# seceq/zkir

Hardware: AMD Instinct MI355X
Metric: trace rows/sec (2^20-cycle fib: execution-trace fill + BabyBear NTT/LDE + Poseidon2 Merkle commitment) (higher is better)
Workload: dtype u32 (Baby Bear, 31-bit modular) / u64 trace words

## Files before the change

### zkir_amd/csrc/babybear.h

```cpp
#pragma once
#include <cstdint>

#if defined(__HIPCC__)
#define BB_HD __host__ __device__ __forceinline__
#else
#define BB_HD inline
#endif

namespace bb {

constexpr uint32_t P = 0x78000001u;
constexpr uint32_t NEG_PINV = 0x77FFFFFFu;
constexpr uint32_t R1 = 0x0FFFFFFEu;
constexpr uint32_t R2 = 0x45DDDDE3u;
constexpr uint32_t GEN = 31u;
constexpr uint32_t ROOT27 = 0x1A427A41u;
constexpr uint32_t W_EXT = 11u;

BB_HD uint32_t add(uint32_t a, uint32_t b) { const uint32_t s = a + b, d = s - P; return d < s ? d : s; }
BB_HD uint32_t sub(uint32_t a, uint32_t b) { const uint32_t d = a - b, e = d + P; return e < d ? e : d; }
BB_HD uint32_t neg(uint32_t a) { return a ? P - a : 0u; }
BB_HD uint32_t dbl(uint32_t a) { return add(a, a); }
BB_HD uint32_t mont_mul(uint32_t a, uint32_t b) {
  const uint64_t t = (uint64_t)a * b;
// ... 179 lines not shown
      "v_mad_i64_i32 %2, vcc, %11, %16, %3\n\tv_mad_i64_i32 %6, vcc, %15, %16, %7\n\t"
      "v_mad_i64_i32 %1, vcc, %9, %17, %1\n\tv_mad_i64_i32 %5, vcc, %13, %17, %5\n\t"
      "v_mad_i64_i32 %3, vcc, %11, %17, %3\n\tv_mad_i64_i32 %7, vcc, %15, %17, %7"
      : "=&v"(ay0), "=&v"(ay1), "=&v"(at2), "=&v"(at3), "=&v"(by0), "=&v"(by1), "=&v"(bt2), "=&v"(bt3)
      : "v"(a[0]), "v"(a[1]), "v"(a[2]), "v"(a[3]), "v"(b[0]), "v"(b[1]), "v"(b[2]), "v"(b[3]), "v"(w1), "v"(n1), "s"(W_ONE) : "vcc");
  {
    const int32_t m0 = (int32_t)((uint32_t)at2 * NEG_PINV), m1 = (int32_t)((uint32_t)bt2 * NEG_PINV), m2 = (int32_t)((uint32_t)at3 * NEG_PINV), m3 = (int32_t)((uint32_t)bt3 * NEG_PINV);
    asm("v_mad_i64_i32 %0, vcc, %4, %8, %0\n\tv_mad_i64_i32 %1, vcc, %5, %8, %1\n\tv_mad_i64_i32 %2, vcc, %6, %8, %2\n\tv_mad_i64_i32 %3, vcc, %7, %8, %3"
        : "+v"(at2), "+v"(bt2), "+v"(at3), "+v"(bt3) : "v"(m0), "v"(m1), "v"(m2), "v"(m3), "s"((int32_t)P) : "vcc");
  }
  const int32_t ay2 = (int32_t)((uint64_t)at2 >> 32), ay3 = (int32_t)((uint64_t)at3 >> 32), by2 = (int32_t)((uint64_t)bt2 >> 32), by3 = (int32_t)((uint64_t)bt3 >> 32);
  int64_t au0, au1, bu0, bu1;
  asm("v_mad_i64_i32 %0, vcc, %8, %12, %4\n\tv_mad_i64_i32 %2, vcc, %10, %12, %6\n\t"
      "v_mad_i64_i32 %1, vcc, %9, %14, %5\n\tv_mad_i64_i32 %3, vcc, %11, %14, %7\n\t"
      "v_mad_i64_i32 %4, vcc, %8, %13, %4\n\tv_mad_i64_i32 %6, vcc, %10, %13, %6\n\t"
      "v_mad_i64_i32 %5, vcc, %9, %15, %5\n\tv_mad_i64_i32 %7, vcc, %11, %15, %7"
      : "=&v"(au0), "=&v"(au1), "=&v"(bu0), "=&v"(bu1), "+v"(ay0), "+v"(ay1), "+v"(by0), "+v"(by1)
      : "v"(ay2), "v"(ay3), "v"(by2), "v"(by3), "v"(w2), "v"(n2), "v"(w2i), "v"(n2i) : "vcc");
  {
    const int32_t m0 = (int32_t)((uint32_t)au0 * NEG_PINV), m1 = (int32_t)((uint32_t)bu0 * NEG_PINV), m2 = (int32_t)((uint32_t)au1 * NEG_PINV), m3 = (int32_t)((uint32_t)bu1 * NEG_PINV);
    const int32_t m4 = (int32_t)((uint32_t)ay0 * NEG_PINV), m5 = (int32_t)((uint32_t)by0 * NEG_PINV), m6 = (int32_t)((uint32_t)ay1 * NEG_PINV), m7 = (int32_t)((uint32_t)by1 * NEG_PINV);
    asm("v_mad_i64_i32 %0, vcc, %8, %16, %0\n\tv_mad_i64_i32 %1, vcc, %9, %16, %1\n\tv_mad_i64_i32 %2, vcc, %10, %16, %2\n\tv_mad_i64_i32 %3, vcc, %11, %16, %3\n\t"
        "v_mad_i64_i32 %4, vcc, %12, %16, %4\n\tv_mad_i64_i32 %5, vcc, %13, %16, %5\n\tv_mad_i64_i32 %6, vcc, %14, %16, %6\n\tv_mad_i64_i32 %7, vcc, %15, %16, %7"
        : "+v"(au0), "+v"(bu0), "+v"(au1), "+v"(bu1), "+v"(ay0), "+v"(by0), "+v"(ay1), "+v"(by1)
        : "v"(m0), "v"(m1), "v"(m2), "v"(m3), "v"(m4), "v"(m5), "v"(m6), "v"(m7), "s"((int32_t)P) : "vcc");
  }
  a[0] = (int32_t)((uint64_t)au0 >> 32); a[1] = (int32_t)((uint64_t)au1 >> 32); a[2] = (int32_t)((uint64_t)ay0 >> 32); a[3] = (int32_t)((uint64_t)ay1 >> 32);
  b[0] = (int32_t)((uint64_t)bu0 >> 32); b[1] = (int32_t)((uint64_t)bu1 >> 32); b[2] = (int32_t)((uint64_t)by0 >> 32); b[3] = (int32_t)((uint64_t)by1 >> 32);
#else
  dit4w(a[0], a[1], a[2], a[3], w1, n1, w2, n2, w2i, n2i);
  dit4w(b[0], b[1], b[2], b[3], w1, n1, w2, n2, w2i, n2i);
#endif
}
constexpr uint64_t WREDC_IN_MAX = (1ull << 63) - ((uint64_t)P << 31);
constexpr uint64_t wredc_out_bound(uint64_t acc) { return (acc >> 32) + 1 + P / 2 + 1; }
struct WBound { uint64_t acc, out; };
constexpr WBound dit2w_bound(uint64_t x) { const uint64_t a = x * (uint64_t)W_ONE + x * (uint64_t)W_HALF; return WBound{a, wredc_out_bound(a)}; }
constexpr WBound dit4w_bound(uint64_t x) {
  const uint64_t s1 = x * (uint64_t)W_ONE + x * (uint64_t)W_HALF;
  const uint64_t s2 = s1 + wredc_out_bound(s1) * (uint64_t)W_HALF;
  return WBound{s2, wredc_out_bound(s2)};
}
static_assert(dit4w_bound(1ull << 31).acc < WREDC_IN_MAX && dit2w_bound(1ull << 31).acc < WREDC_IN_MAX, "every sum of a quad on int32 words is a legal reduction input");
static_assert(dit4w_bound(1ull << 31).out < (1ull << 31) && dit2w_bound(1ull << 31).out < (1ull << 31), "any quad output (and any canonical word) is a legal quad input");
static_assert(dit4w_bound(P).out < P && dit2w_bound(P).out < P, "closure: words in (-p, p) -- canonical ones included -- stay in (-p, p), which is what wcanon() takes");

BB_HD uint32_t to_mont(uint32_t a) { return mont_mul(a, R2); }
BB_HD uint32_t from_mont(uint32_t a) { return mont_mul(a, 1u); }
BB_HD uint32_t mul(uint32_t a, uint32_t b) { return mont_mul(mont_mul(a, b), R2); }
BB_HD uint32_t pow(uint32_t a, uint64_t e) {
  uint32_t r = R1, b = to_mont(a);
  while (e) { if (e & 1) r = mont_mul(r, b); b = mont_mul(b, b); e >>= 1; }
  return from_mont(r);
}
BB_HD uint32_t inv(uint32_t a) { return pow(a, P - 2); }
BB_HD uint32_t root_of_unity(int log_n) { uint32_t w = ROOT27; for (int i = log_n; i < 27; i++) w = mul(w, w); return w; }

struct E4 { uint32_t c[4]; };
BB_HD E4 e_add(const E4& a, const E4& b) { return E4{{add(a.c[0], b.c[0]), add(a.c[1], b.c[1]), add(a.c[2], b.c[2]), add(a.c[3], b.c[3])}}; }
BB_HD E4 e_sub(const E4& a, const E4& b) { return E4{{sub(a.c[0], b.c[0]), sub(a.c[1], b.c[1]), sub(a.c[2], b.c[2]), sub(a.c[3], b.c[3])}}; }
BB_HD E4 e_mul_m(const E4& a, const E4& b) {
  constexpr uint32_t W11M = (uint32_t)((11ull * R1) % P);
  const uint32_t a0 = a.c[0], a1 = a.c[1], a2 = a.c[2], a3 = a.c[3], b0 = b.c[0], b1 = b.c[1], b2 = b.c[2], b3 = b.c[3];
  const uint32_t t4 = add(add(mont_mul(a1, b3), mont_mul(a2, b2)), mont_mul(a3, b1));
  const uint32_t t5 = add(mont_mul(a2, b3), mont_mul(a3, b2));
  const uint32_t t6 = mont_mul(a3, b3);
  E4 r;
  r.c[0] = add(mont_mul(a0, b0), mont_mul(W11M, t4));
  r.c[1] = add(add(mont_mul(a0, b1), mont_mul(a1, b0)), mont_mul(W11M, t5));
  r.c[2] = add(add(add(mont_mul(a0, b2), mont_mul(a1, b1)), mont_mul(a2, b0)), mont_mul(W11M, t6));
  r.c[3] = add(add(mont_mul(a0, b3), mont_mul(a1, b2)), add(mont_mul(a2, b1), mont_mul(a3, b0)));
  return r;
}
BB_HD E4 e_mul_fm(const E4& a, uint32_t bm) { return E4{{mont_mul(a.c[0], bm), mont_mul(a.c[1], bm), mont_mul(a.c[2], bm), mont_mul(a.c[3], bm)}}; }
BB_HD E4 e_to_mont(const E4& a) { return E4{{to_mont(a.c[0]), to_mont(a.c[1]), to_mont(a.c[2]), to_mont(a.c[3])}}; }
BB_HD E4 e_from_mont(const E4& a) { return E4{{from_mont(a.c[0]), from_mont(a.c[1]), from_mont(a.c[2]), from_mont(a.c[3])}}; }
BB_HD E4 e_one_m() { return E4{{R1, 0, 0, 0}}; }
BB_HD E4 e_zero() { return E4{{0, 0, 0, 0}}; }
// ... 17 lines not shown
```

### zkir_amd/csrc/ntt.hip

```cpp
#include <hip/hip_runtime.h>

#include <atomic>
#include <cstdlib>
#include <mutex>
#include <type_traits>

#include "../../include/zkir_amd.h"
#include "../../include/zkir_amd_experimental.h"
#include "babybear.h"
#include "host.h"

namespace {

constexpr int NT = 256;
__device__ __forceinline__ uint32_t bitrev(uint32_t x, int bits) { return bits == 0 ? 0u : __brev(x) >> (32 - bits); }

template <int K, int N, class F>
__device__ __forceinline__ void static_for(F&& f) {
  if constexpr (K < N) { f(std::integral_constant<int, K>{}); static_for<K + 1, N>(f); }
}

using u32x4 = uint32_t __attribute__((ext_vector_type(4)));
__device__ __forceinline__ u32x4 ld4(const uint4* p) { return *reinterpret_cast<const u32x4*>(p); }
__device__ __forceinline__ void st4(uint4* p, u32x4 v) { *reinterpret_cast<u32x4*>(p) = v; }

__device__ __forceinline__ void wave_sync_lds() { asm volatile("s_waitcnt lgkmcnt(0)" ::: "memory"); }

__device__ __forceinline__ uint4 add4(uint4 a, uint4 b) { return make_uint4(bb::add(a.x, b.x), bb::add(a.y, b.y), bb::add(a.z, b.z), bb::add(a.w, b.w)); }
__device__ __forceinline__ uint4 subl4(uint4 a, uint4 b) { return make_uint4(a.x - b.x + bb::P, a.y - b.y + bb::P, a.z - b.z + bb::P, a.w - b.w + bb::P); }
__device__ __forceinline__ uint4 mul4(uint4 a, uint32_t w) { return make_uint4(bb::mont_mul(a.x, w), bb::mont_mul(a.y, w), bb::mont_mul(a.z, w), bb::mont_mul(a.w, w)); }

__device__ __forceinline__ void dif4(uint4& x0, uint4& x1, uint4& x2, uint4& x3, uint32_t wA, uint32_t wB, uint32_t w2) {
  const uint4 y0 = add4(x0, x2), y2 = mul4(subl4(x0, x2), wA);
  const uint4 y1 = add4(x1, x3), y3 = mul4(subl4(x1, x3), wB);
  x0 = add4(y0, y1); x1 = mul4(subl4(y0, y1), w2);
  x2 = add4(y2, y3); x3 = mul4(subl4(y2, y3), w2);
}

struct WTw { int32_t w, n; };
__device__ __forceinline__ WTw wtw(int32_t w) { return WTw{w, -w}; }
__device__ __forceinline__ void dit4w4(uint4& x0, uint4& x1, uint4& x2, uint4& x3, WTw w1, WTw w2, WTw w2i) {
#define ZKIR_Q(c, e) { int32_t a[4] = {(int32_t)x0.c, (int32_t)x1.c, (int32_t)x2.c, (int32_t)x3.c}, b[4] = {(int32_t)x0.e, (int32_t)x1.e, (int32_t)x2.e, (int32_t)x3.e}; \
                       bb::dit4w2(a, b, w1.w, w1.n, w2.w, w2.n, w2i.w, w2i.n); \
                       x0.c = (uint32_t)a[0]; x1.c = (uint32_t)a[1]; x2.c = (uint32_t)a[2]; x3.c = (uint32_t)a[3]; x0.e = (uint32_t)b[0]; x1.e = (uint32_t)b[1]; x2.e = (uint32_t)b[2]; x3.e = (uint32_t)b[3]; }
  ZKIR_Q(x, y) __builtin_amdgcn_sched_barrier(0); ZKIR_Q(z, w)
#undef ZKIR_Q
}
__device__ __forceinline__ void dit2w4(uint4& a, uint4& b, WTw w) {
#define ZKIR_Q(c) { int32_t p = (int32_t)a.c, q = (int32_t)b.c; bb::dit2w(p, q, w.w, w.n); a.c = (uint32_t)p; b.c = (uint32_t)q; }
  ZKIR_Q(x) ZKIR_Q(y) ZKIR_Q(z) ZKIR_Q(w)
#undef ZKIR_Q
}
__device__ __forceinline__ uint4 canon4(uint4 v) { return make_uint4(bb::wcanon((int32_t)v.x), bb::wcanon((int32_t)v.y), bb::wcanon((int32_t)v.z), bb::wcanon((int32_t)v.w)); }

template <bool DIT>
__global__ __launch_bounds__(NT) void ntt_stage_kernel(uint4* __restrict__ data, uint64_t blk_u4, int L, int s0, const uint32_t* __restrict__ tw, int canon) {
  uint4* x = data + (uint64_t)blockIdx.y * blk_u4;
  const uint64_t item = (uint64_t)blockIdx.x * NT + threadIdx.x;
  const uint32_t n = 1u << L;
  if (item >= (uint64_t)n) return;
  const uint32_t t = (uint32_t)(item >> 1), h = (uint32_t)(item & 1);
  uint32_t p, stride, w;
  if (DIT) { stride = 1u << s0; const uint32_t hi = t >> s0, lo = t & (stride - 1); p = (hi << (s0 + 1)) + lo; w = tw[lo << (L - s0 - 1)]; }
  else { stride = n >> (s0 + 1); const uint32_t hi = t / stride, lo = t % stride; p = hi * (n >> s0) + lo; w = tw[lo << s0]; }
  const uint4 a = x[(uint64_t)p * 2 + h], b = x[(uint64_t)(p + stride) * 2 + h];
  if (DIT) {
    uint4 a2 = a, b2 = b;
    dit2w4(a2, b2, wtw(bb::centre(w)));
    if (canon) { a2 = canon4(a2); b2 = canon4(b2); }
    x[(uint64_t)p * 2 + h] = a2; x[(uint64_t)(p + stride) * 2 + h] = b2;
  }
  else { x[(uint64_t)p * 2 + h] = add4(a, b); x[(uint64_t)(p + stride) * 2 + h] = mul4(subl4(a, b), w); }
}

struct TraceSrc01 { zkir_trace_columns t; uint64_t n_real; };
__device__ __forceinline__ u32x4 trace_quad01(const TraceSrc01& q, uint32_t blk, uint32_t half, uint64_t i) {
  const bool pad = i >= q.n_real;
  const uint64_t src = pad ? q.n_real - 1 : i;
  u32x4 r;
  if (blk == 0 && half == 0) {
    const uint64_t pcv = q.t.pc[src];
    r.x = (uint32_t)((q.t.cycle[src] + (i - src)) % bb::P); r.y = (uint32_t)(pcv & 0xFFFFF); r.z = (uint32_t)((pcv >> 20) & 0xFFFFF); r.w = (uint32_t)(pcv >> 40);
  } else if (blk == 0) {
    const uint32_t w = q.t.instruction[src];
    r.x = w & 0x7F; r.y = (w >> 7) & 0xF; r.z = (w >> 11) & 0xF; r.w = (w >> 15) & 0xF;
  } else {
    auto limbs = [&](int g, uint32_t out[3]) {
      const uint64_t o = (uint64_t)g * q.t.reg_stride + src;
      const uint64_t v = q.t.registers[o];
      const int bits = q.t.reg_state[o] ? 30 : 20;
      const uint64_t mask = (1ull << bits) - 1;
      out[0] = (uint32_t)(v & mask); out[1] = (uint32_t)((v >> bits) & mask); out[2] = (uint32_t)(v >> (2 * bits));
    };
    uint32_t a[3], b[3];
    if (half == 0) { limbs(1, a); r.x = q.t.instruction[src] >> 19; r.y = a[0]; r.z = a[1]; r.w = a[2]; }
    else { limbs(2, a); limbs(3, b); r.x = a[0]; r.y = a[1]; r.z = a[2]; r.w = b[0]; }
  }
  return r;
}

template <bool DIT, int R, int C, int NTH, bool FUSED = false>
__global__ __launch_bounds__(NTH) void ntt_strided_r4_kernel(uint4* __restrict__ data, uint64_t blk_u4, uint32_t tiles_per_block, uint32_t total, int L, int s0,
                                                              const uint32_t* __restrict__ tw, const uint32_t* __restrict__ small, int log_small, uint32_t j4_m, int canon, TraceSrc01 fsrc = TraceSrc01{}) {
  constexpr int B = 2 * R;
  constexpr uint32_t POS = 1u << (B + C), QUADS = POS / 4, CMASK = (1u << C) - 1, PLANE = POS + 4;
  constexpr uint32_t MOVES = 2 * POS / NTH;
  static_assert(QUADS % NTH == 0 && NTH % (1 << C) == 0 && (2 * POS) % NTH == 0, "tile / thread geometry");
  extern __shared__ uint4 lds4[];
  const uint32_t n = 1u << L;
  const uint32_t stride_mid = DIT ? (1u << s0) : (n >> (s0 + B));
  const uint32_t lo_tiles = stride_mid >> C;
  auto geometry = [&](uint32_t w, uint4*& x, uint32_t& base, uint32_t& lo0) {
    const uint32_t tile = w % tiles_per_block;
    x = data + (uint64_t)(w / tiles_per_block) * blk_u4;
    const uint32_t hi = tile / lo_tiles;
    lo0 = (tile % lo_tiles) << C;
    base = (DIT ? (hi << (s0 + B)) : hi * (n >> s0)) + lo0;
  };
  static_assert(QUADS == NTH, "one quad per lane and round");
  u32x4 pre[MOVES];
  uint4* x; uint32_t base, lo0;
  uint32_t w = blockIdx.x;
  if (w >= total) return;
  uint32_t sm[R];
#pragma unroll
  for (int r = 0; r < R; r++) {
    const int b = 2 * r;
    const uint32_t qq = threadIdx.x >> C;
    if (!DIT) { const int lg = B - 2 - b; sm[r] = small[(qq & ((1u << lg) - 1)) << (log_small - (B - b))]; }
    else sm[r] = small[(qq & ((1u << b) - 1)) << (log_small - (b + 2))];
  }
  geometry(w, x, base, lo0);
  static_for<0, (int)MOVES>([&](auto kc) {
    constexpr uint32_t k = decltype(kc)::value;
    const uint32_t e = threadIdx.x + k * NTH, row = e >> (C + 1), wv = e & ((2u << C) - 1);
    if constexpr (FUSED) pre[k] = trace_quad01(fsrc, w / tiles_per_block, wv & 1, (uint64_t)base + (uint64_t)row * stride_mid + (wv >> 1));
    else pre[k] = ld4(&x[((uint64_t)base + (uint64_t)row * stride_mid) * 2 + wv]);
  });
  uint32_t tw_cur = DIT ? tw[(lo0 + (threadIdx.x & CMASK)) << (L - s0 - B)] : tw[(lo0 + (threadIdx.x & CMASK)) << s0];
  for (;;) {
    static_for<0, (int)MOVES>([&](auto kc) {
      constexpr uint32_t k = decltype(kc)::value;
      const uint32_t e = threadIdx.x + k * NTH, row = e >> (C + 1), wv = e & ((2u << C) - 1);
      st4(&lds4[(wv & 1) * PLANE + ((row << C) | (wv >> 1))], pre[k]);
    });
    uint32_t tp[R];
    if (DIT) {
      uint32_t u = tw_cur;
#pragma unroll
      for (int r = R - 1; r >= 0; r--) { tp[r] = u; u = bb::mont_mul(u, u); u = bb::mont_mul(u, u); }
    } else {
      uint32_t u = tw_cur;
#pragma unroll
      for (int r = 0; r < R; r++) { tp[r] = u; u = bb::mont_mul(u, u); u = bb::mont_mul(u, u); }
    }
    __syncthreads();
    const uint32_t wn = w + gridDim.x;
    uint4* xn = x; uint32_t base_n = base, lo0_n = lo0;
    if (wn < total) {
      geometry(wn, xn, base_n, lo0_n);
      static_for<0, (int)MOVES>([&](auto kc) {
        constexpr uint32_t k = decltype(kc)::value;
        const uint32_t e = threadIdx.x + k * NTH, row = e >> (C + 1), wv = e & ((2u << C) - 1);
        if constexpr (FUSED) pre[k] = trace_quad01(fsrc, wn / tiles_per_block, wv & 1, (uint64_t)base_n + (uint64_t)row * stride_mid + (wv >> 1));
        else pre[k] = ld4(&xn[((uint64_t)base_n + (uint64_t)row * stride_mid) * 2 + wv]);
      });
      tw_cur = DIT ? tw[(lo0_n + (threadIdx.x & CMASK)) << (L - s0 - B)] : tw[(lo0_n + (threadIdx.x & CMASK)) << s0];
    }
#pragma unroll
    for (int r = 0; r < R; r++) {
      const int b = 2 * r;
#pragma unroll
      for (uint32_t k = 0; k < QUADS / NTH; k++) {
        uint32_t q = threadIdx.x + k * NTH;
        if constexpr (DIT) asm volatile("" : "+v"(q));
        const uint32_t lo_l = q & CMASK, qq = q >> C;
        uint4* pl0 = lds4; uint4* pl1 = lds4 + PLANE;
        if constexpr (!DIT) {
          const int lg = B - 2 - b;
          const uint32_t h2 = 1u << lg, mid_lo = qq & (h2 - 1), mid_hi = qq >> lg;
          const uint32_t i0 = ((((mid_hi << (lg + 2)) | mid_lo)) << C) | lo_l, d = h2 << C;
          const uint32_t wa = bb::mont_mul(tp[r], sm[r]);
          const uint32_t wb = bb::mont_mul(wa, j4_m), wc = bb::mont_mul(wa, wa);
          uint4 x0 = pl0[i0], x1 = pl0[i0 + d], x2 = pl0[i0 + 2 * d], x3 = pl0[i0 + 3 * d];
          uint4 y0 = pl1[i0], y1 = pl1[i0 + d], y2 = pl1[i0 + 2 * d], y3 = pl1[i0 + 3 * d];
          dif4(x0, x1, x2, x3, wa, wb, wc);
          pl0[i0] = x0; pl0[i0 + d] = x1; pl0[i0 + 2 * d] = x2; pl0[i0 + 3 * d] = x3;
          dif4(y0, y1, y2, y3, wa, wb, wc);
          pl1[i0] = y0; pl1[i0 + d] = y1; pl1[i0 + 2 * d] = y2; pl1[i0 + 3 * d] = y3;
        } else {
          const uint32_t dm = 1u << b, mid_lo = qq & (dm - 1), mid_hi = qq >> b;
          const uint32_t i0 = ((((mid_hi << (b + 2)) | mid_lo)) << C) | lo_l, d = dm << C;
          const WTw w2 = wtw(bb::mont_mul_centred(tp[r], sm[r]));
          const uint32_t w2u = bb::wcanon(w2.w);
          const WTw w1 = wtw(bb::mont_mul_centred(w2u, w2u)), w2i = wtw(bb::mont_mul_centred(w2u, j4_m));
          uint4 x0 = pl0[i0], x1 = pl0[i0 + d], x2 = pl0[i0 + 2 * d], x3 = pl0[i0 + 3 * d];
          dit4w4(x0, x1, x2, x3, w1, w2, w2i);
          pl0[i0] = x0; pl0[i0 + d] = x1; pl0[i0 + 2 * d] = x2; pl0[i0 + 3 * d] = x3;
          __builtin_amdgcn_sched_barrier(0);
          uint4 y0 = pl1[i0], y1 = pl1[i0 + d], y2 = pl1[i0 + 2 * d], y3 = pl1[i0 + 3 * d];
          dit4w4(y0, y1, y2, y3, w1, w2, w2i);
          pl1[i0] = y0; pl1[i0 + d] = y1; pl1[i0 + 2 * d] = y2; pl1[i0 + 3 * d] = y3;
        }
      }
      const bool wave_local = !DIT ? (r + 1 < R && B - 2 - b <= 6 - C) : (r + 1 < R && b + 2 <= 6 - C);
      if (wave_local) wave_sync_lds(); else __syncthreads();
    }
#pragma unroll
    for (uint32_t k = 0; k < MOVES; k++) {
      const uint32_t e = threadIdx.x + k * NTH, row = e >> (C + 1), wv = e & ((2u << C) - 1);
      uint4 v = lds4[(wv & 1) * PLANE + ((row << C) | (wv >> 1))];
      if (DIT && canon) v = canon4(v);
      x[((uint64_t)base + (uint64_t)row * stride_mid) * 2 + wv] = v;
    }
    if (wn >= total) break;
    w = wn; x = xn; base = base_n; lo0 = lo0_n;
  }
}

template <bool DIT, int S>
__global__ __launch_bounds__(NT) void ntt_reg_kernel(uint4* __restrict__ data, uint64_t blk_u4, int L, int s0, const uint32_t* __restrict__ tw, uint32_t r4_m, uint32_t r8_m,
                                                       uint32_t r8_3_m, int canon) {
  constexpr int E = 1 << S;
  const uint32_t n = 1u << L;
  uint4* x = data + (uint64_t)blockIdx.y * blk_u4;
  const uint64_t item = (uint64_t)blockIdx.x * NT + threadIdx.x;
  if (item >= ((uint64_t)n >> S) * 2) return;
  const uint32_t t = (uint32_t)(item >> 1), h = (uint32_t)(item & 1);
  const uint32_t d = DIT ? (1u << s0) : (n >> (s0 + S));
  const uint32_t hi = t / d, lo = t % d;
  const uint64_t base = ((uint64_t)hi * d * E + lo) * 2 + h;
  uint4 v[E];
#pragma unroll
  for (int k = 0; k < E; k++) v[k] = x[base + (uint64_t)k * d * 2];
  if (!DIT) {
    const uint32_t T0 = tw[lo << s0];
    const uint32_t T1 = bb::mont_mul(T0, T0);
    if (S == 3) {
      const uint32_t T2 = bb::mont_mul(T1, T1);
      const uint32_t a1 = bb::mont_mul(T0, r8_m), a2 = bb::mont_mul(T0, r4_m), a3 = bb::mont_mul(T0, r8_3_m), b1 = bb::mont_mul(T1, r4_m);
      const uint32_t w0[4] = {T0, a1, a2, a3};
#pragma unroll
      for (int k = 0; k < 4; k++) { const uint4 a = v[k], b = v[k + 4]; v[k] = add4(a, b); v[k + 4] = mul4(subl4(a, b), w0[k]); }
#pragma unroll
      for (int g = 0; g < 8; g += 4) {
        { const uint4 a = v[g], b = v[g + 2]; v[g] = add4(a, b); v[g + 2] = mul4(subl4(a, b), T1); }
        { const uint4 a = v[g + 1], b = v[g + 3]; v[g + 1] = add4(a, b); v[g + 3] = mul4(subl4(a, b), b1); }
      }
#pragma unroll
      for (int g = 0; g < 8; g += 2) { const uint4 a = v[g], b = v[g + 1]; v[g] = add4(a, b); v[g + 1] = mul4(subl4(a, b), T2); }
    } else {
      const uint32_t a1 = bb::mont_mul(T0, r4_m);
      { const uint4 a = v[0], b = v[2]; v[0] = add4(a, b); v[2] = mul4(subl4(a, b), T0); }
      { const uint4 a = v[1], b = v[3]; v[1] = add4(a, b); v[3] = mul4(subl4(a, b), a1); }
#pragma unroll
      for (int g = 0; g < 4; g += 2) { const uint4 a = v[g], b = v[g + 1]; v[g] = add4(a, b); v[g + 1] = mul4(subl4(a, b), T1); }
    }
  } else {
    const uint32_t Uf = tw[lo << (L - s0 - S)];
    const uint32_t Um = bb::mont_mul(Uf, Uf);
    if (S == 3) {
      const WTw u0 = wtw(bb::mont_mul_centred(Um, Um)), um = wtw(bb::centre(Um)), m1 = wtw(bb::mont_mul_centred(Um, r4_m));
#pragma unroll
      for (int g = 0; g < 8; g += 4) dit4w4(v[g], v[g + 1], v[g + 2], v[g + 3], u0, um, m1);
      const WTw wf[4] = {wtw(bb::centre(Uf)), wtw(bb::mont_mul_centred(Uf, r8_m)), wtw(bb::mont_mul_centred(Uf, r4_m)), wtw(bb::mont_mul_centred(Uf, r8_3_m))};
#pragma unroll
      for (int k = 0; k < 4; k++) dit2w4(v[k], v[k + 4], wf[k]);
    } else {
      dit4w4(v[0], v[1], v[2], v[3], wtw(bb::centre(Um)), wtw(bb::centre(Uf)), wtw(bb::mont_mul_centred(Uf, r4_m)));
    }
    if (canon) {
#pragma unroll
      for (int k = 0; k < E; k++) v[k] = canon4(v[k]);
    }
  }
#pragma unroll
  for (int k = 0; k < E; k++) x[base + (uint64_t)k * d * 2] = v[k];
}

inline unsigned cu_count() {
  static std::mutex mu;
  static unsigned cached[64] = {};
  int dev = 0;
  if (hipGetDevice(&dev) != hipSuccess || dev < 0 || dev >= 64) return 256u;
  std::lock_guard<std::mutex> lk(mu);
  if (!cached[dev]) { hipDeviceProp_t p; cached[dev] = hipGetDeviceProperties(&p, dev) == hipSuccess && p.multiProcessorCount > 0 ? (unsigned)p.multiProcessorCount : 256u; }
  return cached[dev];
}
inline int persist() { static const int v = getenv("ZKIR_NTT_PERSIST") ? atoi(getenv("ZKIR_NTT_PERSIST")) : 1; return v; }
// ... 64 lines not shown
      const uint32_t half = 1u << hb;
      for (uint32_t q = threadIdx.x; q < (n >> 1); q += NT) {
        const uint32_t r_lo = q & (half - 1), r_hi = q >> hb;
        const uint32_t ia = (r_hi << (hb + 1)) | r_lo, ib = ia + half;
        const uint32_t a = lds[ia], bv = lds[ib];
        lds[ia] = bb::add(a, bv); lds[ib] = bb::mont_mul(bb::sub(a, bv), small_inv[r_lo << b]);
      }
      __syncthreads();
    }
    uint32_t v[2];
    int cnt = 0;
    for (uint32_t e = threadIdx.x; e < n; e += NT) { const uint32_t k = bitrev(e, L); v[cnt++] = bb::mont_mul(bb::mont_mul(lds[e], g_lo[k & 1023]), g_hi[k >> 10]); }
    __syncthreads();
    cnt = 0;
    for (uint32_t e = threadIdx.x; e < n; e += NT) { lds[2 * e] = v[cnt]; lds[2 * e + 1] = v[cnt]; cnt++; }
    __syncthreads();
    for (int s = 1; s <= L; s++) {
      const uint32_t half = 1u << s;
      for (uint32_t q = threadIdx.x; q < n; q += NT) {
        const uint32_t r_lo = q & (half - 1), r_hi = q >> s;
        const uint32_t ia = (r_hi << (s + 1)) | r_lo, ib = ia + half;
        const uint32_t a = lds[ia], t = bb::mont_mul(lds[ib], small_fwd[r_lo << (L - s)]);
        lds[ia] = bb::add(a, t); lds[ib] = bb::sub(a, t);
      }
      __syncthreads();
    }
    for (uint32_t e = threadIdx.x; e < 2 * n; e += NT) y[(uint64_t)e * 8 + c] = lds[e];
    __syncthreads();
  }
}

constexpr int MID_NT = 512;
__global__ __launch_bounds__(MID_NT) __attribute__((amdgpu_waves_per_eu(4, 4))) void lde_middle_r4_kernel(const uint4* __restrict__ in, uint4* __restrict__ out, uint32_t chunks_per_block, uint32_t total, int L,
                                                                const uint32_t* __restrict__ small_inv, const uint32_t* __restrict__ small_fwd,
                                                                const uint32_t* __restrict__ g_lo, const uint32_t* __restrict__ g_hi, uint32_t j4_inv_m, uint32_t j4_fwd_m, int canon) {
  constexpr int Bm = 10;
  constexpr uint32_t APL = 1024;
  __shared__ uint4 A[2 * APL];
  __shared__ uint4 Bf[2048];
  const uint32_t n = 1u << L, t = threadIdx.x;
  uint32_t w = blockIdx.x;
  if (w >= total) return;
  uint32_t tw_i[5], tw_f[5];
#pragma unroll
  for (int r = 0; r < 5; r++) {
    const int lg = 8 - 2 * r;
    tw_i[r] = small_inv[((t & 255) & ((1u << lg) - 1)) << (2 * r)];
    const int sft = 2 * r + 1;
    tw_f[r] = small_fwd[(t & ((1u << sft) - 1)) << (Bm - sft - 1)];
  }
  u32x4 pre[4];
  uint32_t glo[4], ghi[4];
  auto fetch = [&](uint32_t ww) {
    const uint4* x = in + ((uint64_t)(ww / chunks_per_block) * n + ((uint64_t)(ww % chunks_per_block) << Bm)) * 2;
#pragma unroll
    for (int k = 0; k < 4; k++) pre[k] = ld4(&x[t + k * MID_NT]);
    const uint32_t p0 = ((ww % chunks_per_block) << Bm) + 4 * (t & 255);
#pragma unroll
    for (int i = 0; i < 4; i++) { const uint32_t k = bitrev(p0 + i, L); glo[i] = g_lo[k & 1023]; ghi[i] = g_hi[k >> 10]; }
  };
  fetch(w);
  for (;;) {
    const uint32_t base = (w % chunks_per_block) << Bm;
    uint4* y = out + (uint64_t)(w / chunks_per_block) * n * 4;
#pragma unroll
    for (int k = 0; k < 4; k++) { const uint32_t e = t + k * MID_NT; st4(&A[(e & 1) * APL + (e >> 1)], pre[k]); }
    uint32_t gs[4];
#pragma unroll
    for (int i = 0; i < 4; i++) gs[i] = bb::mont_mul(glo[i], ghi[i]);
    __syncthreads();
    const uint32_t wn = w + gridDim.x;
    if (wn < total) fetch(wn);
    {
      const uint32_t q = t & 255;
      uint4* a = A + (t >> 8) * APL;
#pragma unroll
      for (int r = 0; r < 5; r++) {
        const int lg = 8 - 2 * r;
        const uint32_t h2 = 1u << lg, lo = q & (h2 - 1), hi = q >> lg;
        const uint32_t i0 = (hi << (lg + 2)) | lo;
        const uint32_t wA = tw_i[r];
        const uint32_t wB = bb::mont_mul(wA, j4_inv_m), w2 = bb::mont_mul(wA, wA);
        uint4 x0 = a[i0], x1 = a[i0 + h2], x2 = a[i0 + 2 * h2], x3 = a[i0 + 3 * h2];
        dif4(x0, x1, x2, x3, wA, wB, w2);
        if (r == 4) {
          x0 = mul4(x0, gs[0]); x1 = mul4(x1, gs[1]); x2 = mul4(x2, gs[2]); x3 = mul4(x3, gs[3]);
        }
        a[i0] = x0; a[i0 + h2] = x1; a[i0 + 2 * h2] = x2; a[i0 + 3 * h2] = x3;
        if (r >= 1 && r < 4) wave_sync_lds(); else __syncthreads();
      }
    }
#pragma unroll 1
    for (int h = 0; h < 2; h++) {
      const uint4* a = A + h * APL;
      uint4* F = h == 0 ? Bf : A;
#pragma unroll
      for (int r = 0; r < 5; r++) {
        const int s = 2 * r + 1;
        const uint32_t lo = t & ((1u << s) - 1), hi = t >> s;
        const uint32_t i0 = (hi << (s + 2)) | lo, d = 1u << s;
        const uint32_t w2 = tw_f[r];
        const WTw c2 = wtw(bb::centre(w2)), c1 = wtw(bb::mont_mul_centred(w2, w2)), c2i = wtw(bb::mont_mul_centred(w2, j4_fwd_m));
        uint4 x0, x1, x2, x3;
        if (r == 0) {
          x0 = a[i0 >> 1]; x1 = a[(i0 + d) >> 1]; x2 = a[(i0 + 2 * d) >> 1]; x3 = a[(i0 + 3 * d) >> 1];
          __syncthreads();
        } else { x0 = F[i0]; x1 = F[i0 + d]; x2 = F[i0 + 2 * d]; x3 = F[i0 + 3 * d]; }
        dit4w4(x0, x1, x2, x3, c1, c2, c2i);
        F[i0] = x0; F[i0 + d] = x1; F[i0 + 2 * d] = x2; F[i0 + 3 * d] = x3;
        if (r < 2) wave_sync_lds(); else __syncthreads();
      }
    }
#pragma unroll
    for (int k = 0; k < 4; k++) {
      const uint32_t e = t + k * MID_NT;
      uint4 v0 = Bf[e], v1 = A[e];
      if (canon) { v0 = canon4(v0); v1 = canon4(v1); }
      y[((uint64_t)2 * base + e) * 2] = v0; y[((uint64_t)2 * base + e) * 2 + 1] = v1;
    }
    __syncthreads();
    if (wn >= total) break;
    w = wn;
  }
}

}

namespace zkir {

void lde_run(const LdeTables& t, uint32_t* in, uint32_t n_blocks, uint32_t* out, void* stream) {
  hipStream_t s = (hipStream_t)stream;
  const int L = t.log_n;
  const uint32_t N = 1u << L;
  static const uint32_t j4_inv_m = bb::to_mont(bb::inv(bb::root_of_unity(2))), j4_fwd_m = bb::to_mont(bb::root_of_unity(2));
  static const uint32_t r8_fwd = bb::root_of_unity(3), r8_inv = bb::inv(r8_fwd);
  static const uint32_t r8_inv_m = bb::to_mont(r8_inv), r8_inv3_m = bb::to_mont(bb::mul(bb::mul(r8_inv, r8_inv), r8_inv));
  static const uint32_t r8_fwd_m = bb::to_mont(r8_fwd), r8_fwd3_m = bb::to_mont(bb::mul(bb::mul(r8_fwd, r8_fwd), r8_fwd));
  if (L < 10) {
    hipLaunchKernelGGL(lde_small_kernel, dim3(n_blocks), dim3(NT), (8u << L), s, in, out, L, t.small_inv, t.small_fwd, t.g_lo, t.g_hi);
    return;
  }
  run_strided_stages<false>(in, N, n_blocks, L, 0, L - 10, t.tw_inv, t.small_inv, 10, j4_inv_m, r8_inv_m, r8_inv3_m, s);
  {
    const uint32_t chunks = N >> 10, total = chunks * n_blocks;
    unsigned grid = persist() ? cu_count() * 2 : total;
    if (grid > total) grid = total;
    hipLaunchKernelGGL(lde_middle_r4_kernel, dim3(grid), dim3(MID_NT), 0, s, (const uint4*)in, (uint4*)out, chunks, total, L, t.small_inv, t.small_fwd, t.g_lo, t.g_hi,
                       j4_inv_m, j4_fwd_m, L == 10);
  }
  run_strided_stages<true>(out, (uint64_t)2 * N, n_blocks, L + 1, 11, L - 10, t.tw_fwd, t.small_fwd, 11, j4_fwd_m, r8_fwd_m, r8_fwd3_m, s);
}


bool strided_variant_run(const LdeTables& t, uint32_t* data, uint32_t n_blocks, int variant, bool dit, void* stream) {
  hipStream_t s = (hipStream_t)stream;
  const int L = dit ? t.log_n + 1 : t.log_n;
  if (t.log_n < 20) return false;
  const uint64_t n = (uint64_t)1 << L;
  static const uint32_t j4_inv_m = bb::to_mont(bb::inv(bb::root_of_unity(2))), j4_fwd_m = bb::to_mont(bb::root_of_unity(2));
  const uint32_t* tw = dit ? t.tw_fwd : t.tw_inv; const uint32_t* sm = dit ? t.small_fwd : t.small_inv;
  const int ls = dit ? 11 : 10; const uint32_t j4 = dit ? j4_fwd_m : j4_inv_m; const int s0 = dit ? 11 : 0;
#define ZKIR_VARIANT(R, C, NTH) do { if (dit) launch_strided_r4<true, R, C, NTH>(data, n, n_blocks, L, s0, tw, sm, ls, j4, s); else launch_strided_r4<false, R, C, NTH>(data, n, n_blocks, L, s0, tw, sm, ls, j4, s); } while (0)
  switch (variant) {
    case 0: ZKIR_VARIANT(5, 2, 1024); break;
    case 1: ZKIR_VARIANT(5, 1, 512); break;
    case 2: ZKIR_VARIANT(4, 3, 512); break;
    case 3: ZKIR_VARIANT(4, 2, 256); break;
    case 4: ZKIR_VARIANT(3, 4, 256); break;
    default: return false;
  }
#undef ZKIR_VARIANT
  return true;
}

bool lde_run_fused01(const LdeTables& t, const zkir_trace_columns* trace, uint64_t n_real, uint32_t* in, uint32_t n_blocks, uint32_t* out, void* stream) {
  hipStream_t s = (hipStream_t)stream;
  const int L = t.log_n;
  if (L < 20 || L == 21 || n_blocks < 3 || strided_c() != 2) return false;
  const uint32_t N = 1u << L;
  static const uint32_t j4_inv_m = bb::to_mont(bb::inv(bb::root_of_unity(2))), j4_fwd_m = bb::to_mont(bb::root_of_unity(2));
  static const uint32_t r8_fwd = bb::root_of_unity(3), r8_inv = bb::inv(r8_fwd);
  static const uint32_t r8_inv_m = bb::to_mont(r8_inv), r8_inv3_m = bb::to_mont(bb::mul(bb::mul(r8_inv, r8_inv), r8_inv));
  static const uint32_t r8_fwd_m = bb::to_mont(r8_fwd), r8_fwd3_m = bb::to_mont(bb::mul(bb::mul(r8_fwd, r8_fwd), r8_fwd));
  const TraceSrc01 src{*trace, n_real};
  launch_strided_r4<false, 5, 2, 1024, true>(in, N, 2, L, 0, t.tw_inv, t.small_inv, 10, j4_inv_m, s, &src);
  launch_strided_r4<false, 5, 2, 1024>(in + (uint64_t)2 * N * 8, N, n_blocks - 2, L, 0, t.tw_inv, t.small_inv, 10, j4_inv_m, s);
  if (L - 10 > 10) run_strided_stages<false>(in, N, n_blocks, L, 10, L - 20, t.tw_inv, t.small_inv, 10, j4_inv_m, r8_inv_m, r8_inv3_m, s);
  {
    const uint32_t chunks = N >> 10, total = chunks * n_blocks;
    unsigned grid = persist() ? cu_count() * 2 : total;
    if (grid > total) grid = total;
    hipLaunchKernelGGL(lde_middle_r4_kernel, dim3(grid), dim3(MID_NT), 0, s, (const uint4*)in, (uint4*)out, chunks, total, L, t.small_inv, t.small_fwd, t.g_lo, t.g_hi,
                       j4_inv_m, j4_fwd_m, L == 10);
  }
  run_strided_stages<true>(out, (uint64_t)2 * N, n_blocks, L + 1, 11, L - 10, t.tw_fwd, t.small_fwd, 11, j4_fwd_m, r8_fwd_m, r8_fwd3_m, s);
  return true;
}

}
```

Measured before the change: 188.0 million.

## Switch inverse NTT stages from Gentleman-Sande DIF to signed-word Cooley-Tukey quads

The inverse (DIF) path of the strided, radix-8/4 and middle LDE kernels now uses Cooley-Tukey butterflies on signed centred words (ct4w4/dit2w4 with the v_mad_i64_i32 reduction) instead of the unsigned Montgomery add/sub/mul dif4. Twiddles are indexed by bit-reversed block index, so each tile loads its per-round factors from the twiddle table rather than squaring tw_cur repeatedly. The coset scale in the middle kernel uses a new vectorised signed scale. The goal is to reuse the cheaper lazy-reduction quad on the inverse side too, at the cost of an extra table argument, per-tile twiddle gathers, and new bound assertions that correctness depends on.

```diff
diff --git a/zkir_amd/csrc/babybear.h b/zkir_amd/csrc/babybear.h
--- a/zkir_amd/csrc/babybear.h
+++ b/zkir_amd/csrc/babybear.h
@@ -235,6 +235,28 @@
   dit4w(b[0], b[1], b[2], b[3], w1, n1, w2, n2, w2i, n2i);
 #endif
 }
+BB_HD void ct4w(int32_t& x0, int32_t& x1, int32_t& x2, int32_t& x3, int32_t w1, int32_t n1, int32_t w2, int32_t n2, int32_t w2i, int32_t n2i) {
+  dit4w(x0, x2, x1, x3, w1, n1, w2, n2, w2i, n2i);
+}
+BB_HD void ct4w2(int32_t* a, int32_t* b, int32_t w1, int32_t n1, int32_t w2, int32_t n2, int32_t w2i, int32_t n2i) {
+  int32_t p[4] = {a[0], a[2], a[1], a[3]}, q[4] = {b[0], b[2], b[1], b[3]};
+  dit4w2(p, q, w1, n1, w2, n2, w2i, n2i);
+  a[0] = p[0]; a[1] = p[2]; a[2] = p[1]; a[3] = p[3]; b[0] = q[0]; b[1] = q[2]; b[2] = q[1]; b[3] = q[3];
+}
+BB_HD int32_t wscale(int32_t x, uint32_t g) { return wredc(wmul(x, (int32_t)g)); }
+BB_HD void wscale4(int32_t* x, uint32_t g) {
+#if defined(__HIP_DEVICE_COMPILE__)
+  int64_t t0, t1, t2, t3;
+  asm("v_mad_i64_i32 %0, vcc, %4, %8, 0\n\tv_mad_i64_i32 %1, vcc, %5, %8, 0\n\tv_mad_i64_i32 %2, vcc, %6, %8, 0\n\tv_mad_i64_i32 %3, vcc, %7, %8, 0"
+      : "=&v"(t0), "=&v"(t1), "=&v"(t2), "=&v"(t3) : "v"(x[0]), "v"(x[1]), "v"(x[2]), "v"(x[3]), "v"(g) : "vcc");
+  const int32_t m0 = (int32_t)((uint32_t)t0 * NEG_PINV), m1 = (int32_t)((uint32_t)t1 * NEG_PINV), m2 = (int32_t)((uint32_t)t2 * NEG_PINV), m3 = (int32_t)((uint32_t)t3 * NEG_PINV);
+  asm("v_mad_i64_i32 %0, vcc, %4, %8, %0\n\tv_mad_i64_i32 %1, vcc, %5, %8, %1\n\tv_mad_i64_i32 %2, vcc, %6, %8, %2\n\tv_mad_i64_i32 %3, vcc, %7, %8, %3"
+      : "+v"(t0), "+v"(t1), "+v"(t2), "+v"(t3) : "v"(m0), "v"(m1), "v"(m2), "v"(m3), "s"((int32_t)P) : "vcc");
+  x[0] = (int32_t)((uint64_t)t0 >> 32); x[1] = (int32_t)((uint64_t)t1 >> 32); x[2] = (int32_t)((uint64_t)t2 >> 32); x[3] = (int32_t)((uint64_t)t3 >> 32);
+#else
+  for (int i = 0; i < 4; i++) x[i] = wscale(x[i], g);
+#endif
+}
 constexpr uint64_t WREDC_IN_MAX = (1ull << 63) - ((uint64_t)P << 31);
 constexpr uint64_t wredc_out_bound(uint64_t acc) { return (acc >> 32) + 1 + P / 2 + 1; }
 struct WBound { uint64_t acc, out; };
@@ -247,6 +269,11 @@
 static_assert(dit4w_bound(1ull << 31).acc < WREDC_IN_MAX && dit2w_bound(1ull << 31).acc < WREDC_IN_MAX, "every sum of a quad on int32 words is a legal reduction input");
 static_assert(dit4w_bound(1ull << 31).out < (1ull << 31) && dit2w_bound(1ull << 31).out < (1ull << 31), "any quad output (and any canonical word) is a legal quad input");
 static_assert(dit4w_bound(P).out < P && dit2w_bound(P).out < P, "closure: words in (-p, p) -- canonical ones included -- stay in (-p, p), which is what wcanon() takes");
+constexpr WBound ct4w_bound(uint64_t x) { return dit4w_bound(x); }
+constexpr WBound wscale_bound(uint64_t x) { const uint64_t a = x * (uint64_t)(P - 1); return WBound{a, wredc_out_bound(a)}; }
+static_assert(ct4w_bound(1ull << 31).acc < WREDC_IN_MAX && ct4w_bound(1ull << 31).out < (1ull << 31), "every sum of an inverse quad on int32 words is a legal reduction input, every output a legal input");
+static_assert(ct4w_bound(P).out < P, "closure of the inverse rounds: canonical words and words in (-p, p) stay in (-p, p)");
+static_assert(wscale_bound(P).acc < WREDC_IN_MAX && wscale_bound(P).out < P, "the coset scale of a word in (-p, p) is a word in (-p, p): the forward rounds take it as it is");
 
 BB_HD uint32_t to_mont(uint32_t a) { return mont_mul(a, R2); }
 BB_HD uint32_t from_mont(uint32_t a) { return mont_mul(a, 1u); }
diff --git a/zkir_amd/csrc/ntt.hip b/zkir_amd/csrc/ntt.hip
--- a/zkir_amd/csrc/ntt.hip
+++ b/zkir_amd/csrc/ntt.hip
@@ -25,17 +25,6 @@
 __device__ __forceinline__ void st4(uint4* p, u32x4 v) { *reinterpret_cast<u32x4*>(p) = v; }
 
 __device__ __forceinline__ void wave_sync_lds() { asm volatile("s_waitcnt lgkmcnt(0)" ::: "memory"); }
-
-__device__ __forceinline__ uint4 add4(uint4 a, uint4 b) { return make_uint4(bb::add(a.x, b.x), bb::add(a.y, b.y), bb::add(a.z, b.z), bb::add(a.w, b.w)); }
-__device__ __forceinline__ uint4 subl4(uint4 a, uint4 b) { return make_uint4(a.x - b.x + bb::P, a.y - b.y + bb::P, a.z - b.z + bb::P, a.w - b.w + bb::P); }
-__device__ __forceinline__ uint4 mul4(uint4 a, uint32_t w) { return make_uint4(bb::mont_mul(a.x, w), bb::mont_mul(a.y, w), bb::mont_mul(a.z, w), bb::mont_mul(a.w, w)); }
-
-__device__ __forceinline__ void dif4(uint4& x0, uint4& x1, uint4& x2, uint4& x3, uint32_t wA, uint32_t wB, uint32_t w2) {
-  const uint4 y0 = add4(x0, x2), y2 = mul4(subl4(x0, x2), wA);
-  const uint4 y1 = add4(x1, x3), y3 = mul4(subl4(x1, x3), wB);
-  x0 = add4(y0, y1); x1 = mul4(subl4(y0, y1), w2);
-  x2 = add4(y2, y3); x3 = mul4(subl4(y2, y3), w2);
-}
 
 struct WTw { int32_t w, n; };
 __device__ __forceinline__ WTw wtw(int32_t w) { return WTw{w, -w}; }
@@ -45,6 +34,18 @@
                        x0.c = (uint32_t)a[0]; x1.c = (uint32_t)a[1]; x2.c = (uint32_t)a[2]; x3.c = (uint32_t)a[3]; x0.e = (uint32_t)b[0]; x1.e = (uint32_t)b[1]; x2.e = (uint32_t)b[2]; x3.e = (uint32_t)b[3]; }
   ZKIR_Q(x, y) __builtin_amdgcn_sched_barrier(0); ZKIR_Q(z, w)
 #undef ZKIR_Q
+}
+__device__ __forceinline__ void ct4w4(uint4& x0, uint4& x1, uint4& x2, uint4& x3, WTw w1, WTw w2, WTw w2i) { dit4w4(x0, x2, x1, x3, w1, w2, w2i); }
+__device__ __forceinline__ void ct_twiddles(uint32_t sm, uint32_t f, bool unit, uint32_t j4_m, WTw& w1, WTw& w2, WTw& w2i) {
+  uint32_t w2u;
+  if (unit) { w2u = sm; w2 = wtw(bb::centre(sm)); }
+  else { w2 = wtw(bb::mont_mul_centred(sm, f)); w2u = bb::wcanon(w2.w); }
+  w1 = wtw(bb::mont_mul_centred(w2u, w2u)); w2i = wtw(bb::mont_mul_centred(w2u, j4_m));
+}
+__device__ __forceinline__ uint4 scale4(uint4 v, uint32_t g) {
+  int32_t x[4] = {(int32_t)v.x, (int32_t)v.y, (int32_t)v.z, (int32_t)v.w};
+  bb::wscale4(x, g);
+  return make_uint4((uint32_t)x[0], (uint32_t)x[1], (uint32_t)x[2], (uint32_t)x[3]);
 }
 __device__ __forceinline__ void dit2w4(uint4& a, uint4& b, WTw w) {
 #define ZKIR_Q(c) { int32_t p = (int32_t)a.c, q = (int32_t)b.c; bb::dit2w(p, q, w.w, w.n); a.c = (uint32_t)p; b.c = (uint32_t)q; }
@@ -62,15 +63,11 @@
   const uint32_t t = (uint32_t)(item >> 1), h = (uint32_t)(item & 1);
   uint32_t p, stride, w;
   if (DIT) { stride = 1u << s0; const uint32_t hi = t >> s0, lo = t & (stride - 1); p = (hi << (s0 + 1)) + lo; w = tw[lo << (L - s0 - 1)]; }
-  else { stride = n >> (s0 + 1); const uint32_t hi = t / stride, lo = t % stride; p = hi * (n >> s0) + lo; w = tw[lo << s0]; }
-  const uint4 a = x[(uint64_t)p * 2 + h], b = x[(uint64_t)(p + stride) * 2 + h];
-  if (DIT) {
-    uint4 a2 = a, b2 = b;
-    dit2w4(a2, b2, wtw(bb::centre(w)));
-    if (canon) { a2 = canon4(a2); b2 = canon4(b2); }
-    x[(uint64_t)p * 2 + h] = a2; x[(uint64_t)(p + stride) * 2 + h] = b2;
-  }
-  else { x[(uint64_t)p * 2 + h] = add4(a, b); x[(uint64_t)(p + stride) * 2 + h] = mul4(subl4(a, b), w); }
+  else { stride = n >> (s0 + 1); const uint32_t hi = t / stride, lo = t % stride; p = hi * (n >> s0) + lo; w = tw[bitrev(hi, s0) << (L - s0 - 1)]; }
+  uint4 a = x[(uint64_t)p * 2 + h], b = x[(uint64_t)(p + stride) * 2 + h];
+  dit2w4(a, b, wtw(bb::centre(w)));
+  if (DIT && canon) { a = canon4(a); b = canon4(b); }
+  x[(uint64_t)p * 2 + h] = a; x[(uint64_t)(p + stride) * 2 + h] = b;
 }
 
 struct TraceSrc01 { zkir_trace_columns t; uint64_t n_real; };
@@ -110,16 +107,16 @@
   const uint32_t n = 1u << L;
   const uint32_t stride_mid = DIT ? (1u << s0) : (n >> (s0 + B));
   const uint32_t lo_tiles = stride_mid >> C;
-  auto geometry = [&](uint32_t w, uint4*& x, uint32_t& base, uint32_t& lo0) {
+  auto geometry = [&](uint32_t w, uint4*& x, uint32_t& base, uint32_t& lo0, uint32_t& hi) {
     const uint32_t tile = w % tiles_per_block;
     x = data + (uint64_t)(w / tiles_per_block) * blk_u4;
-    const uint32_t hi = tile / lo_tiles;
+    hi = tile / lo_tiles;
     lo0 = (tile % lo_tiles) << C;
     base = (DIT ? (hi << (s0 + B)) : hi * (n >> s0)) + lo0;
   };
   static_assert(QUADS == NTH, "one quad per lane and round");
   u32x4 pre[MOVES];
-  uint4* x; uint32_t base, lo0;
+  uint4* x; uint32_t base, lo0, hi;
   uint32_t w = blockIdx.x;
   if (w >= total) return;
   uint32_t sm[R];
@@ -127,17 +124,27 @@
   for (int r = 0; r < R; r++) {
     const int b = 2 * r;
     const uint32_t qq = threadIdx.x >> C;
-    if (!DIT) { const int lg = B - 2 - b; sm[r] = small[(qq & ((1u << lg) - 1)) << (log_small - (B - b))]; }
+    if (!DIT) sm[r] = small[bitrev(qq >> (B - 2 - b), b) << (log_small - (b + 2))];
     else sm[r] = small[(qq & ((1u << b) - 1)) << (log_small - (b + 2))];
   }
-  geometry(w, x, base, lo0);
+  const bool unit = s0 == 0;
+  uint32_t tf_next[R] = {};
+  auto tile_factors = [&](uint32_t hi_t) {
+    if (DIT || unit) return;
+    const uint32_t e = bitrev(hi_t, s0);
+#pragma unroll
+    for (int r = 0; r < R; r++) tf_next[r] = tw[e << (L - s0 - 2 * r - 2)];
+  };
+  geometry(w, x, base, lo0, hi);
   static_for<0, (int)MOVES>([&](auto kc) {
     constexpr uint32_t k = decltype(kc)::value;
     const uint32_t e = threadIdx.x + k * NTH, row = e >> (C + 1), wv = e & ((2u << C) - 1);
     if constexpr (FUSED) pre[k] = trace_quad01(fsrc, w / tiles_per_block, wv & 1, (uint64_t)base + (uint64_t)row * stride_mid + (wv >> 1));
     else pre[k] = ld4(&x[((uint64_t)base + (uint64_t)row * stride_mid) * 2 + wv]);
   });
-  uint32_t tw_cur = DIT ? tw[(lo0 + (threadIdx.x & CMASK)) << (L - s0 - B)] : tw[(lo0 + (threadIdx.x & CMASK)) << s0];
+  uint32_t tw_cur = 0;
+  if (DIT) tw_cur = tw[(lo0 + (threadIdx.x & CMASK)) << (L - s0 - B)];
+  tile_factors(hi);
   for (;;) {
     static_for<0, (int)MOVES>([&](auto kc) {
       constexpr uint32_t k = decltype(kc)::value;
@@ -150,22 +157,22 @@
 #pragma unroll
       for (int r = R - 1; r >= 0; r--) { tp[r] = u; u = bb::mont_mul(u, u); u = bb::mont_mul(u, u); }
     } else {
-      uint32_t u = tw_cur;
-#pragma unroll
-      for (int r = 0; r < R; r++) { tp[r] = u; u = bb::mont_mul(u, u); u = bb::mont_mul(u, u); }
+#pragma unroll
+      for (int r = 0; r < R; r++) tp[r] = tf_next[r];
     }
     __syncthreads();
     const uint32_t wn = w + gridDim.x;
-    uint4* xn = x; uint32_t base_n = base, lo0_n = lo0;
+    uint4* xn = x; uint32_t base_n = base, lo0_n = lo0, hi_n = hi;
     if (wn < total) {
-      geometry(wn, xn, base_n, lo0_n);
+      geometry(wn, xn, base_n, lo0_n, hi_n);
       static_for<0, (int)MOVES>([&](auto kc) {
         constexpr uint32_t k = decltype(kc)::value;
         const uint32_t e = threadIdx.x + k * NTH, row = e >> (C + 1), wv = e & ((2u << C) - 1);
         if constexpr (FUSED) pre[k] = trace_quad01(fsrc, wn / tiles_per_block, wv & 1, (uint64_t)base_n + (uint64_t)row * stride_mid + (wv >> 1));
         else pre[k] = ld4(&xn[((uint64_t)base_n + (uint64_t)row * stride_mid) * 2 + wv]);
       });
-      tw_cur = DIT ? tw[(lo0_n + (threadIdx.x & CMASK)) << (L - s0 - B)] : tw[(lo0_n + (threadIdx.x & CMASK)) << s0];
+      if (DIT) tw_cur = tw[(lo0_n + (threadIdx.x & CMASK)) << (L - s0 - B)];
+      tile_factors(hi_n);
     }
 #pragma unroll
     for (int r = 0; r < R; r++) {
@@ -173,20 +180,21 @@
 #pragma unroll
       for (uint32_t k = 0; k < QUADS / NTH; k++) {
         uint32_t q = threadIdx.x + k * NTH;
-        if constexpr (DIT) asm volatile("" : "+v"(q));
+        asm volatile("" : "+v"(q));
         const uint32_t lo_l = q & CMASK, qq = q >> C;
         uint4* pl0 = lds4; uint4* pl1 = lds4 + PLANE;
         if constexpr (!DIT) {
           const int lg = B - 2 - b;
           const uint32_t h2 = 1u << lg, mid_lo = qq & (h2 - 1), mid_hi = qq >> lg;
           const uint32_t i0 = ((((mid_hi << (lg + 2)) | mid_lo)) << C) | lo_l, d = h2 << C;
-          const uint32_t wa = bb::mont_mul(tp[r], sm[r]);
-          const uint32_t wb = bb::mont_mul(wa, j4_m), wc = bb::mont_mul(wa, wa);
+          WTw w1, w2, w2i;
+          ct_twiddles(sm[r], tp[r], unit, j4_m, w1, w2, w2i);
           uint4 x0 = pl0[i0], x1 = pl0[i0 + d], x2 = pl0[i0 + 2 * d], x3 = pl0[i0 + 3 * d];
+          ct4w4(x0, x1, x2, x3, w1, w2, w2i);
+          pl0[i0] = x0; pl0[i0 + d] = x1; pl0[i0 + 2 * d] = x2; pl0[i0 + 3 * d] = x3;
+          __builtin_amdgcn_sched_barrier(0);
           uint4 y0 = pl1[i0], y1 = pl1[i0 + d], y2 = pl1[i0 + 2 * d], y3 = pl1[i0 + 3 * d];
-          dif4(x0, x1, x2, x3, wa, wb, wc);
-          pl0[i0] = x0; pl0[i0 + d] = x1; pl0[i0 + 2 * d] = x2; pl0[i0 + 3 * d] = x3;
-          dif4(y0, y1, y2, y3, wa, wb, wc);
+          ct4w4(y0, y1, y2, y3, w1, w2, w2i);
           pl1[i0] = y0; pl1[i0 + d] = y1; pl1[i0 + 2 * d] = y2; pl1[i0 + 3 * d] = y3;
         } else {
           const uint32_t dm = 1u << b, mid_lo = qq & (dm - 1), mid_hi = qq >> b;
@@ -214,7 +222,7 @@
       x[((uint64_t)base + (uint64_t)row * stride_mid) * 2 + wv] = v;
     }
     if (wn >= total) break;
-    w = wn; x = xn; base = base_n; lo0 = lo0_n;
+    w = wn; x = xn; base = base_n; lo0 = lo0_n; hi = hi_n;
   }
 }
 
@@ -234,27 +242,17 @@
 #pragma unroll
   for (int k = 0; k < E; k++) v[k] = x[base + (uint64_t)k * d * 2];
   if (!DIT) {
-    const uint32_t T0 = tw[lo << s0];
-    const uint32_t T1 = bb::mont_mul(T0, T0);
+    const uint32_t Tf = tw[bitrev(hi, s0) << (L - s0 - S)];
+    const uint32_t Tm = bb::mont_mul(Tf, Tf);
     if (S == 3) {
-      const uint32_t T2 = bb::mont_mul(T1, T1);
-      const uint32_t a1 = bb::mont_mul(T0, r8_m), a2 = bb::mont_mul(T0, r4_m), a3 = bb::mont_mul(T0, r8_3_m), b1 = bb::mont_mul(T1, r4_m);
-      const uint32_t w0[4] = {T0, a1, a2, a3};
-#pragma unroll
-      for (int k = 0; k < 4; k++) { const uint4 a = v[k], b = v[k + 4]; v[k] = add4(a, b); v[k + 4] = mul4(subl4(a, b), w0[k]); }
-#pragma unroll
-      for (int g = 0; g < 8; g += 4) {
-        { const uint4 a = v[g], b = v[g + 2]; v[g] = add4(a, b); v[g + 2] = mul4(subl4(a, b), T1); }
-        { const uint4 a = v[g + 1], b = v[g + 3]; v[g + 1] = add4(a, b); v[g + 3] = mul4(subl4(a, b), b1); }
-      }
-#pragma unroll
-      for (int g = 0; g < 8; g += 2) { const uint4 a = v[g], b = v[g + 1]; v[g] = add4(a, b); v[g + 1] = mul4(subl4(a, b), T2); }
+      const WTw t0 = wtw(bb::mont_mul_centred(Tm, Tm)), tm = wtw(bb::centre(Tm)), m1 = wtw(bb::mont_mul_centred(Tm, r4_m));
+#pragma unroll
+      for (int g = 0; g < 2; g++) ct4w4(v[g], v[g + 2], v[g + 4], v[g + 6], t0, tm, m1);
+      const WTw wf[4] = {wtw(bb::centre(Tf)), wtw(bb::mont_mul_centred(Tf, r4_m)), wtw(bb::mont_mul_centred(Tf, r8_m)), wtw(bb::mont_mul_centred(Tf, r8_3_m))};
+#pragma unroll
+      for (int m = 0; m < 4; m++) dit2w4(v[2 * m], v[2 * m + 1], wf[m]);
     } else {
-      const uint32_t a1 = bb::mont_mul(T0, r4_m);
-      { const uint4 a = v[0], b = v[2]; v[0] = add4(a, b); v[2] = mul4(subl4(a, b), T0); }
-      { const uint4 a = v[1], b = v[3]; v[1] = add4(a, b); v[3] = mul4(subl4(a, b), a1); }
-#pragma unroll
-      for (int g = 0; g < 4; g += 2) { const uint4 a = v[g], b = v[g + 1]; v[g] = add4(a, b); v[g + 1] = mul4(subl4(a, b), T1); }
+      ct4w4(v[0], v[1], v[2], v[3], wtw(bb::centre(Tm)), wtw(bb::centre(Tf)), wtw(bb::mont_mul_centred(Tf, r4_m)));
     }
   } else {
     const uint32_t Uf = tw[lo << (L - s0 - S)];
@@ -385,7 +383,7 @@
 
 constexpr int MID_NT = 512;
 __global__ __launch_bounds__(MID_NT) __attribute__((amdgpu_waves_per_eu(4, 4))) void lde_middle_r4_kernel(const uint4* __restrict__ in, uint4* __restrict__ out, uint32_t chunks_per_block, uint32_t total, int L,
-                                                                const uint32_t* __restrict__ small_inv, const uint32_t* __restrict__ small_fwd,
+                                                                const uint32_t* __restrict__ tw_inv, const uint32_t* __restrict__ small_inv, const uint32_t* __restrict__ small_fwd,
                                                                 const uint32_t* __restrict__ g_lo, const uint32_t* __restrict__ g_hi, uint32_t j4_inv_m, uint32_t j4_fwd_m, int canon) {
   constexpr int Bm = 10;
   constexpr uint32_t APL = 1024;
@@ -398,11 +396,12 @@
 #pragma unroll
   for (int r = 0; r < 5; r++) {
     const int lg = 8 - 2 * r;
-    tw_i[r] = small_inv[((t & 255) & ((1u << lg) - 1)) << (2 * r)];
+    tw_i[r] = small_inv[bitrev((t & 255) >> lg, 2 * r) << lg];
     const int sft = 2 * r + 1;
     tw_f[r] = small_fwd[(t & ((1u << sft) - 1)) << (Bm - sft - 1)];
   }
   u32x4 pre[4];
+  uint32_t cf_next[5];
   uint32_t glo[4], ghi[4];
   auto fetch = [&](uint32_t ww) {
     const uint4* x = in + ((uint64_t)(ww / chunks_per_block) * n + ((uint64_t)(ww % chunks_per_block) << Bm)) * 2;
@@ -411,6 +410,9 @@
     const uint32_t p0 = ((ww % chunks_per_block) << Bm) + 4 * (t & 255);
 #pragma unroll
     for (int i = 0; i < 4; i++) { const uint32_t k = bitrev(p0 + i, L); glo[i] = g_lo[k & 1023]; ghi[i] = g_hi[k >> 10]; }
+    const uint32_t ce = bitrev(ww % chunks_per_block, L - Bm);
+#pragma unroll
+    for (int r = 0; r < 5; r++) cf_next[r] = tw_inv[ce << (8 - 2 * r)];
   };
   fetch(w);
   for (;;) {
@@ -421,6 +423,9 @@
     uint32_t gs[4];
 #pragma unroll
     for (int i = 0; i < 4; i++) gs[i] = bb::mont_mul(glo[i], ghi[i]);
+    uint32_t cf[5];
+#pragma unroll
+    for (int r = 0; r < 5; r++) cf[r] = cf_next[r];
     __syncthreads();
     const uint32_t wn = w + gridDim.x;
     if (wn < total) fetch(wn);
@@ -432,12 +437,12 @@
         const int lg = 8 - 2 * r;
         const uint32_t h2 = 1u << lg, lo = q & (h2 - 1), hi = q >> lg;
         const uint32_t i0 = (hi << (lg + 2)) | lo;
-        const uint32_t wA = tw_i[r];
-        const uint32_t wB = bb::mont_mul(wA, j4_inv_m), w2 = bb::mont_mul(wA, wA);
+        WTw c1, c2, c2i;
+        ct_twiddles(tw_i[r], cf[r], false, j4_inv_m, c1, c2, c2i);
         uint4 x0 = a[i0], x1 = a[i0 + h2], x2 = a[i0 + 2 * h2], x3 = a[i0 + 3 * h2];
-        dif4(x0, x1, x2, x3, wA, wB, w2);
+        ct4w4(x0, x1, x2, x3, c1, c2, c2i);
         if (r == 4) {
-          x0 = mul4(x0, gs[0]); x1 = mul4(x1, gs[1]); x2 = mul4(x2, gs[2]); x3 = mul4(x3, gs[3]);
+          x0 = scale4(x0, gs[0]); x1 = scale4(x1, gs[1]); x2 = scale4(x2, gs[2]); x3 = scale4(x3, gs[3]);
         }
         a[i0] = x0; a[i0 + h2] = x1; a[i0 + 2 * h2] = x2; a[i0 + 3 * h2] = x3;
         if (r >= 1 && r < 4) wave_sync_lds(); else __syncthreads();
@@ -498,7 +503,7 @@
     const uint32_t chunks = N >> 10, total = chunks * n_blocks;
     unsigned grid = persist() ? cu_count() * 2 : total;
     if (grid > total) grid = total;
-    hipLaunchKernelGGL(lde_middle_r4_kernel, dim3(grid), dim3(MID_NT), 0, s, (const uint4*)in, (uint4*)out, chunks, total, L, t.small_inv, t.small_fwd, t.g_lo, t.g_hi,
+    hipLaunchKernelGGL(lde_middle_r4_kernel, dim3(grid), dim3(MID_NT), 0, s, (const uint4*)in, (uint4*)out, chunks, total, L, t.tw_inv, t.small_inv, t.small_fwd, t.g_lo, t.g_hi,
                        j4_inv_m, j4_fwd_m, L == 10);
   }
   run_strided_stages<true>(out, (uint64_t)2 * N, n_blocks, L + 1, 11, L - 10, t.tw_fwd, t.small_fwd, 11, j4_fwd_m, r8_fwd_m, r8_fwd3_m, s);
@@ -543,7 +548,7 @@
     const uint32_t chunks = N >> 10, total = chunks * n_blocks;
     unsigned grid = persist() ? cu_count() * 2 : total;
     if (grid > total) grid = total;
-    hipLaunchKernelGGL(lde_middle_r4_kernel, dim3(grid), dim3(MID_NT), 0, s, (const uint4*)in, (uint4*)out, chunks, total, L, t.small_inv, t.small_fwd, t.g_lo, t.g_hi,
+    hipLaunchKernelGGL(lde_middle_r4_kernel, dim3(grid), dim3(MID_NT), 0, s, (const uint4*)in, (uint4*)out, chunks, total, L, t.tw_inv, t.small_inv, t.small_fwd, t.g_lo, t.g_hi,
                        j4_inv_m, j4_fwd_m, L == 10);
   }
   run_strided_stages<true>(out, (uint64_t)2 * N, n_blocks, L + 1, 11, L - 10, t.tw_fwd, t.small_fwd, 11, j4_fwd_m, r8_fwd_m, r8_fwd3_m, s);
```

Result: faster. 191.2 million, median of 6 (+1.7%).
